# ShMonem/animSnapBases

Hardware: AMD Instinct MI355X
Metric: snapshots/sec (SVD+SPLOCS) for n_verts x n_frames; basis Frobenius err vs ref (higher is better)
Workload: dtype f64

## Files before the change

animsnapbases_amd/_lib.py:

```python
import ctypes
import os

import numpy as np

_HERE = os.path.dirname(os.path.abspath(__file__))
LIB_PATH = os.path.join(_HERE, "libasb_hip.so")

c_dp = ctypes.c_void_p
c_i64 = ctypes.c_int64
c_int = ctypes.c_int
c_dbl = ctypes.c_double

ASB_OK = 0
ERR_LIMIT = -4
DEFLATE_RESIDUAL, DEFLATE_PROJECT = 0, 1

PROTOTYPES = {
    "asb_abi_version": (c_int, []),
    "asb_create": (c_int, [c_int, ctypes.c_void_p, ctypes.POINTER(ctypes.c_void_p)]),
    "asb_destroy": (None, [ctypes.c_void_p]),
    "asb_last_error": (ctypes.c_char_p, [ctypes.c_void_p]),
    "asb_sync": (c_int, [ctypes.c_void_p]),
    "asb_prof_reset": (c_int, [ctypes.c_void_p, c_int]),
    "asb_prof_get": (c_int, [ctypes.c_void_p, ctypes.POINTER(c_i64), ctypes.POINTER(c_dbl)]),
# ... 98 lines not shown
    "asb_deflate_download_residual": (c_int, [ctypes.c_void_p, c_dp]),
    "asb_deflate_block_argmax": (c_int, [ctypes.c_void_p, c_int, c_dp, c_dp]),
    "asb_deflate_force_next": (c_int, [ctypes.c_void_p, c_i64]),
    "asb_components_post": (c_int, [ctypes.c_void_p, c_int, c_dbl, c_dp, c_dp]),
    "asb_orth_gram": (c_int, [ctypes.c_void_p, c_dp]),
    "asb_orth_apply": (c_int, [ctypes.c_void_p, c_dp, c_dp]),
    "asb_orth_refine": (c_int, [ctypes.c_void_p, c_dp]),
    "asb_orth_gram_get": (c_int, [ctypes.c_void_p, c_dp]),
    "asb_components_transform": (c_int, [ctypes.c_void_p, c_dp]),
    "asb_components_download": (c_int, [ctypes.c_void_p, c_dp]),
    "asb_components_upload": (c_int, [ctypes.c_void_p, c_dp, c_i64]),
    "asb_geodesic_setup": (c_int, [ctypes.c_void_p, c_int, c_int] + [c_dp] * 14),
    "asb_geodesic_solve": (c_int, [ctypes.c_void_p, c_dp, c_int, c_dbl, c_dp, c_dp]),
    "asb_geodesic_dense_setup": (c_int, [ctypes.c_void_p]),
    "asb_geodesic_bt_setup": (c_int, [ctypes.c_void_p, c_int, c_dp, c_dp, c_dp, c_dp, c_dp, c_dp, c_dp, c_dp]),
    "asb_deflate_apply_geodesic": (c_int, [ctypes.c_void_p, c_i64, c_dbl, c_dbl]),
    "asb_align_frames": (c_int, [ctypes.c_void_p, c_dp, c_i64, c_i64, c_int, c_dp]),
    "asb_pod_gram": (c_int, [ctypes.c_void_p, c_dp, c_dp]),
    "asb_pod_basis": (c_int, [ctypes.c_void_p, c_dp, c_dp, c_i64]),
    "asb_pod_project": (c_int, [ctypes.c_void_p, c_dp, c_dp]),
    "asb_components_truncate": (c_int, [ctypes.c_void_p, c_i64]),
    "asb_sym_tridiag": (c_int, [ctypes.c_void_p, c_dp, c_i64, c_dp, c_dp]),
    "asb_sym_backtransform": (c_int, [ctypes.c_void_p, c_dp, c_i64, c_dp, c_i64, c_dp]),
    "asb_snapshots_affine": (c_int, [ctypes.c_void_p, c_dbl, c_int, c_dp]),
    "asb_qr_apply": (c_int, [ctypes.c_void_p, c_dp]),
    "asb_deim_step": (c_int, [ctypes.c_void_p, c_i64, c_dp, ctypes.POINTER(c_i64), ctypes.POINTER(c_dbl)]),
    "asb_deim_row": (c_int, [ctypes.c_void_p, c_i64, c_dp]),
    "asb_recon_sweep": (c_int, [ctypes.c_void_p, c_int, c_dp, c_i64, c_dp, c_dp, c_dp]),
    "asb_heldout_upload": (c_int, [ctypes.c_void_p, c_dp, c_i64, c_i64, c_i64, c_i64, c_dp, c_int, c_dbl]),
    "asb_heldout_gram": (c_int, [ctypes.c_void_p, c_dp, c_dp]),
    "asb_heldout_factor": (c_int, [ctypes.c_void_p, c_dp, c_dp, ctypes.POINTER(c_i64)]),
    "asb_heldout_weights": (c_int, [ctypes.c_void_p, c_dp]),
    "asb_rows_gather": (c_int, [ctypes.c_void_p, c_int, c_dp, c_i64, c_dp, c_dp]),
    "asb_interp_sweep": (c_int, [ctypes.c_void_p, c_int, c_dp, c_dp, c_i64, c_dp, c_dp, c_i64, c_dp, c_dp, c_dp]),
    "asb_onmesh_mesh": (c_int, [ctypes.c_void_p, c_dp, c_i64, c_dp, c_dp, c_i64, c_i64]),
    "asb_onmesh_run": (c_int, [ctypes.c_void_p, c_int, c_i64, c_i64, c_i64, c_i64, c_int, c_dp, c_int, c_dbl, c_dbl,
                               c_dp, c_dp, c_dp, c_dp, c_dp, c_dp, c_dp]),
    "asb_cproj_setup": (c_int, [ctypes.c_void_p, c_int, c_i64, c_dp, c_dp, c_dp, c_dp]),
    "asb_cproj_run": (c_int, [ctypes.c_void_p, c_int, c_i64, c_i64, c_i64, c_dp, c_int, c_dbl, c_dbl, c_dbl, ctypes.c_void_p]),
    "asb_cforce_run": (c_int, [ctypes.c_void_p, c_int, c_i64, c_i64, c_i64, c_dp, c_int, c_dbl, c_dbl, c_dbl, c_i64, c_dp, c_dp, c_dp,
                               c_int, c_i64, ctypes.c_void_p]),
    "asb_splocs_begin": (c_int, [ctypes.c_void_p]),
    "asb_splocs_gram": (c_int, [ctypes.c_void_p, c_dp, c_dp, ctypes.POINTER(c_dbl)]),
    "asb_splocs_weights": (c_int, [ctypes.c_void_p, c_dp, c_dp, c_dp, c_dp]),
    "asb_splocs_admm": (c_int, [ctypes.c_void_p, c_dp, c_dbl, c_int]),
    "asb_splocs_admm_fields": (c_int, [ctypes.c_void_p, c_dp, c_dbl, c_dbl, c_dbl, c_dbl, c_int]),
    "asb_geodesic_cache_add": (c_int, [ctypes.c_void_p, c_dp, c_int, c_dbl, c_dp]),
    "asb_geodesic_cache_clear": (c_int, [ctypes.c_void_p]),
    "asb_splocs_objective": (c_int, [ctypes.c_void_p, c_dp, c_dp, ctypes.POINTER(c_dbl), ctypes.POINTER(c_dbl),
                                     ctypes.POINTER(c_dbl)]),
    "asb_splocs_results": (c_int, [ctypes.c_void_p, c_dp, c_dp]),
    "asb_test_eig3": (None, [c_dp, c_dp]),
    "asb_test_eig3_fast": (None, [c_dp, c_dp]),
    "asb_test_pick_cfg": (None, [c_i64, c_dp]),
    "asb_test_eig3_dev": (c_int, [ctypes.c_void_p, c_int, c_dp, c_i64, c_dp, c_i64]),
    "asb_test_deflate_step": (c_int, [ctypes.c_void_p, c_i64, c_dp, c_dbl, c_dp]),
    "asb_test_deflate_state": (c_int, [ctypes.c_void_p, c_dp, c_dp, c_dp, c_dp, c_dp, c_dp, c_dp, c_dp]),
    "asb_test_local_best": (c_int, [ctypes.c_void_p, c_i64, c_dp]),
    "asb_test_pick_records": (c_int, [ctypes.c_void_p, c_i64, c_dp, c_i64]),
    "asb_test_sketch_predict": (c_int, [ctypes.c_void_p, c_dp, c_dp, c_dp, c_i64, c_int, c_int, c_dp, ctypes.POINTER(c_i64),
                                        ctypes.POINTER(c_int)]),
    "asb_test_spd_inverse": (c_int, [ctypes.c_void_p, c_dp, c_i64, c_dp]),
    "asb_test_project_columns": (c_int, [ctypes.c_void_p, c_dp, c_i64, c_i64, c_int, c_dp, c_int, c_dp, c_i64]),
    "asb_test_gemm_nn": (c_int, [ctypes.c_void_p, c_dp, c_i64, c_dp, c_i64, c_dp, c_i64, c_i64, c_i64, c_i64, c_dbl, c_dbl, c_int,
                                 c_i64]),
    "asb_test_gemm_tn": (c_int, [ctypes.c_void_p, c_int, c_dp, c_i64, c_i64, c_dp, c_i64, c_i64, c_i64, c_i64, c_dp, c_i64, c_i64,
                                 c_i64, c_i64]),
    "asb_test_transpose": (c_int, [ctypes.c_void_p, c_dp, c_i64, c_i64, c_dp, c_i64]),
    "asb_test_sym_eig": (c_int, [ctypes.c_void_p, c_dp, c_i64, c_dp, c_dp, ctypes.POINTER(c_int)]),
    "asb_test_splocs_install": (c_int, [ctypes.c_void_p, c_dp, c_dp, c_dp]),
    "asb_test_splocs_state": (c_int, [ctypes.c_void_p, c_dp, c_dp, c_dp, c_dp, c_dp]),
    "asb_test_slab_gemm64": (c_int, [ctypes.c_void_p, c_dp, c_i64, c_dp, c_dp, c_i64, c_i64, c_dbl, c_dbl, c_int]),
    "asb_test_geodesic_field1": (c_int, [ctypes.c_void_p, c_i64, c_dp]),
    "asb_test_support_weights": (c_int, [ctypes.c_void_p, c_dp, c_i64, c_i64, c_i64, c_dbl, c_dbl, c_dp]),
    "asb_test_geodesic_cached": (c_int, [ctypes.c_void_p, c_i64, c_dp]),
}


class AsbLibraryError(RuntimeError):
    pass


_lib = None


def _preload_torch_hip_runtime():
    import importlib.util
    import sys
    if "torch" in sys.modules:
        return
    try:
        spec = importlib.util.find_spec("torch")
    except (ImportError, ValueError):
        spec = None
    if spec is None or not spec.origin:
        return
    libdir = os.path.join(os.path.dirname(spec.origin), "lib")
    for name in ("libamdhip64.so", "libamdhip64.so.7", "libamdhip64.so.6"):
        path = os.path.join(libdir, name)
        if os.path.exists(path):
            try:
                ctypes.CDLL(path, mode=ctypes.RTLD_GLOBAL)
            except OSError:
                pass
            return

# ... 35 lines not shown
```

animsnapbases_amd/csrc/asb_deflate.hip:

```cpp
#include "asb_kernels.h"

extern "C" void asb_test_eig3(const double* a6, double* out4) {
    eig3_top(a6[0], a6[1], a6[2], a6[3], a6[4], a6[5], out4[0], out4[1], out4[2], out4[3]);
}
extern "C" void asb_test_eig3_fast(const double* a6, double* out4) {
    eig3_top_fast(a6[0], a6[1], a6[2], a6[3], a6[4], a6[5], out4[0], out4[1], out4[2], out4[3]);
}
extern "C" void asb_test_pick_cfg(int64_t Fp, int* out5) {
    StreamCfg c{0, 0, 0, 0};
    out5[0] = pick_cfg(Fp, c) ? 1 : 0;
    out5[1] = c.T; out5[2] = c.E2; out5[3] = c.block; out5[4] = c.vpb;
}

static int stream_pass(asb_ctx* ctx, bool update, const double* wk, double* scal_k, const double* s,
                       double* ck) {
    StreamCfg c;
    if (!pick_cfg(ctx->Fp, c)) ASB_FAIL(ctx, ASB_ERR_LIMIT, "F = %lld too large (max 32768)", (long long)ctx->F);
    const int grid = stream_grid(ctx, c, ctx->n_loc);
    StreamArgs a{ctx->R, wk, scal_k, s, ck, ctx->energy, ctx->pmax, ctx->pidx, ctx->psum, (long long)ctx->n_loc, nullptr};
    size_t slot;
    int rc = prof_begin(ctx, slot);
    if (rc) return rc;
    launch_stream(ctx, c, update, grid, a);
    ASB_CHECK_LAUNCH(ctx);
    rc = prof_end(ctx, slot);
    if (rc) return rc;
    ctx->nblk = grid;
    return ASB_OK;
}

extern "C" int asb_deflate_begin(asb_ctx* ctx, int64_t K, int mode, int local_support) {
    if (!ctx) return ASB_ERR_ARG;
    if (!ctx->X) ASB_FAIL(ctx, ASB_ERR_ARG, "asb_deflate_begin: no snapshots uploaded");
    if (K < 1) ASB_FAIL(ctx, ASB_ERR_ARG, "asb_deflate_begin: K = %lld", (long long)K);
    if (mode != ASB_DEFLATE_RESIDUAL && mode != ASB_DEFLATE_PROJECT)
        ASB_FAIL(ctx, ASB_ERR_ARG, "asb_deflate_begin: unknown mode %d", mode);
    if (mode == ASB_DEFLATE_PROJECT && local_support)
        ASB_FAIL(ctx, ASB_ERR_ARG, "asb_deflate_begin: the projection mode is only valid for global support");
    ASB_HIP(ctx, hipSetDevice(ctx->dev));
    ctx->K = K;
    ctx->mode = mode;
    ctx->local = local_support;
    ctx->k_done = 0;
    ctx->n_panels = ctx->n_refresh = 0;
    ctx->n_spec_steps = ctx->n_spec_kept = 0;
    ctx->n_guess_panels = 0;
    ctx->n_coop_launches = ctx->max_read_kept = 0;
    ctx->n_sketch_runs = ctx->n_sketch_reads = 0;
    if (ctx->sk_counts) ASB_HIP(ctx, hipMemsetAsync(ctx->sk_counts, 0, 4 * sizeof(unsigned), ctx->stream));
    ctx->sketch_valid = false;
    ctx->sketch_run_off = false;
    ctx->read_by_score = ctx->last_by_score = false;
    ctx->rate_plain = ctx->rate_sketch = -1.0;
    ctx->mode_streak = 0;
    ctx->probe_after = 2;
    ctx->spec_budget = ASB_PANEL_COLS;
    ctx->fb_mark_reads = ctx->fb_mark_k = 0;
    ctx->k_switch = -1;
    {
// ... 376 lines not shown
```

animsnapbases_amd/csrc/asb_kernels.h:

```cpp
#pragma once
#include "asb_common.h"

#include <cmath>
#include <cstdlib>
#include <cstring>



template <int T, int E2, bool UPDATE>
__global__ __launch_bounds__((T >= 256 ? T : 256)) void k_stream(
    double* __restrict__ R, const double* __restrict__ wk, double* __restrict__ scal_k,
    const double* __restrict__ s, double* __restrict__ ck_out, double* __restrict__ energy,
    double* __restrict__ pmax, long long* __restrict__ pidx, double* __restrict__ psum,
    long long n_loc, int F2, const PanelState* __restrict__ panel) {
    if (panel != nullptr) {
        if (panel->done) return;
        if (panel->n_cand < n_loc) n_loc = panel->n_cand;
    }
    constexpr int BLOCK = (T >= 256 ? T : 256);
    constexpr int VPB = BLOCK / T;
    constexpr int NW = T / 64;
    const int tid = threadIdx.x;
    const int g = tid / T, t = tid % T;
    const int wig = t >> 6, lane = tid & 63;
// ... 158 lines not shown
__host__ __device__ inline void eig3_top_fast(double a00, double a01, double a02, double a11, double a12, double a22,
                                              double& lam, double& u0, double& u1, double& u2) {
    const double sc = fmax(fmax(fabs(a00), fabs(a11)), fmax(fabs(a22), fmax(fabs(a01), fmax(fabs(a02), fabs(a12)))));
    if (!(sc > 0.0) || !(sc < 1.0e300)) { eig3_top(a00, a01, a02, a11, a12, a22, lam, u0, u1, u2); return; }
    const double is = 1.0 / sc;
    const double b00 = a00 * is, b01 = a01 * is, b02 = a02 * is, b11 = a11 * is, b12 = a12 * is, b22 = a22 * is;
    const double q = (b00 + b11 + b22) / 3.0;
    const double p1 = b01 * b01 + b02 * b02 + b12 * b12;
    const double d0 = b00 - q, d1 = b11 - q, d2 = b22 - q;
    const double p = sqrt((d0 * d0 + d1 * d1 + d2 * d2 + 2.0 * p1) / 6.0);
    bool ok = p > 0.0;
    double l = q, x = 0.0, y = 0.0, z = 0.0;
    if (ok) {
        const double ip = 1.0 / p;
        const double c00 = d0 * ip, c11 = d1 * ip, c22 = d2 * ip, c01 = b01 * ip, c02 = b02 * ip, c12 = b12 * ip;
        double r = 0.5 * (c00 * (c11 * c22 - c12 * c12) - c01 * (c01 * c22 - c12 * c02) + c02 * (c01 * c12 - c11 * c02));
        r = fmin(1.0, fmax(-1.0, r));
        l = q + 2.0 * p * cos(acos(r) / 3.0);
        for (int it = 0; it < 3 && ok; ++it) {
            const double m00 = b00 - l, m11 = b11 - l, m22 = b22 - l;
            const double x0 = b01 * b12 - b02 * m11, y0 = b02 * b01 - m00 * b12, z0 = m00 * m11 - b01 * b01;
            const double x1 = b01 * m22 - b02 * b12, y1 = b02 * b02 - m00 * m22, z1 = m00 * b12 - b01 * b02;
            const double x2 = m11 * m22 - b12 * b12, y2 = b12 * b02 - b01 * m22, z2 = b01 * b12 - m11 * b02;
            const double n0 = x0 * x0 + y0 * y0 + z0 * z0, n1 = x1 * x1 + y1 * y1 + z1 * z1, n2 = x2 * x2 + y2 * y2 + z2 * z2;
            double nn;
            if (n0 >= n1 && n0 >= n2) { x = x0; y = y0; z = z0; nn = n0; }
            else if (n1 >= n2) { x = x1; y = y1; z = z1; nn = n1; }
            else { x = x2; y = y2; z = z2; nn = n2; }
            if (!(nn > 1.0e-20)) { ok = false; break; }
            const double inn = 1.0 / sqrt(nn);
            x *= inn; y *= inn; z *= inn;
            const double ln = x * (b00 * x + b01 * y + b02 * z) + y * (b01 * x + b11 * y + b12 * z) + z * (b02 * x + b12 * y + b22 * z);
            const bool settled = fabs(ln - l) <= 8.9e-16 * fabs(ln);
            l = ln;
            if (settled) break;
        }
    }
    if (ok) {
        const double r0 = b00 * x + b01 * y + b02 * z - l * x, r1 = b01 * x + b11 * y + b12 * z - l * y,
                     r2 = b02 * x + b12 * y + b22 * z - l * z;
        const double tr = b00 + b11 + b22 - l;
        const double mm = b00 * b11 - b01 * b01 + b00 * b22 - b02 * b02 + b11 * b22 - b12 * b12 - l * tr;
        const double disc = tr * tr - 4.0 * mm;
        const double l2 = 0.5 * (tr + sqrt(fmax(disc, 0.0)));
        ok = fmax(fabs(r0), fmax(fabs(r1), fabs(r2))) <= 1.0e-15 && l2 <= l * (1.0 - 1.0e-6);
    }
    if (!ok) { eig3_top(a00, a01, a02, a11, a12, a22, lam, u0, u1, u2); return; }
    const double m0 = fabs(x), m1 = fabs(y), m2 = fabs(z);
    const double lead = (m0 >= m1 && m0 >= m2) ? x : (m1 >= m2 ? y : z);
    if (lead < 0.0) { x = -x; y = -y; z = -z; }
    lam = l * sc; u0 = x; u1 = y; u2 = z;
}

__device__ inline void reduce_partials(const double* pmax, const long long* pidx, const double* psum,
                                int nblk, double* sh_d, long long* sh_i, double& be, long long& bi,
                                double& bs) {
    const int tid = threadIdx.x, nt = blockDim.x;
    double e = -1.0, s = 0.0;
    long long ix = 0x7fffffffffffffffLL;
    for (int b = tid; b < nblk; b += nt) {
        s += psum[b];
        if (am_better(pmax[b], pidx[b], e, ix)) {
            e = pmax[b];
            ix = pidx[b];
        }
    }
    sh_d[tid] = e;
    sh_d[nt + tid] = s;
    sh_i[tid] = ix;
    __syncthreads();
    for (int o = nt >> 1; o > 0; o >>= 1) {
        if (tid < o) {
            sh_d[nt + tid] += sh_d[nt + tid + o];
            if (am_better(sh_d[tid + o], sh_i[tid + o], sh_d[tid], sh_i[tid])) {
                sh_d[tid] = sh_d[tid + o];
                sh_i[tid] = sh_i[tid + o];
            }
        }
        __syncthreads();
    }
    be = sh_d[0];
    bi = sh_i[0];
    bs = sh_d[nt];
    __syncthreads();
}

static __global__ __launch_bounds__(256) void k_local_best(const double* __restrict__ R,
                                                    const double* pmax, const long long* pidx,
                                                    const double* psum, int nblk, long long v0,
                                                    int Fp, double* __restrict__ rec,
                                                    double* __restrict__ scal, long long k, long long forced,
                                                    long long n_loc) {
    __shared__ double sh_d[512];
    __shared__ long long sh_i[256];
    double be, bs;
    long long bi;
    reduce_partials(pmax, pidx, psum, nblk, sh_d, sh_i, be, bi, bs);
    if (forced >= 0) {
        const bool mine = forced >= v0 && forced < v0 + n_loc;
        be = mine ? 1.0e300 : -1.0;
        bi = mine ? forced - v0 : 0;
    }
    if (threadIdx.x == 0) {
        rec[0] = be;
        rec[1] = __longlong_as_double(v0 + bi);
        if (k > 0) scal[(k - 1) * 4 + 3] = bs;
// ... 217 lines not shown
```

animsnapbases_amd/csrc/asb_project.hip:

```cpp
#include "asb_kernels.h"

#include <algorithm>
#include <atomic>
#include <chrono>
#include <cstdlib>

typedef double d4 __attribute__((ext_vector_type(4)));

#define ASB_NBINS 2048

enum { SC_NORMX2 = 0, SC_E0MAX = 1, SC_EMAX = 2, SC_LO = 3, SC_HI = 4, SC_ABOVE = 5, SC_TAU = 6, SC_OVERFLOW = 7,
       SC_TAU_HI = 11, SC_TAU2 = 12, SC_BANDMAX = 13, SC_TAUG = 16, SC_GG = 24, SC_HH = 32,
       SC_TAU_DIV = 40, SC_DIV_SEED = 41 };
#define ASB_NG 6
__device__ __forceinline__ double guess_score(double ev, double m, double s, double g, double h) { return ev + g * m + h * s; }
__device__ __forceinline__ bool in_guess(double e, double ev, const double* __restrict__ sc) {
    const double m = e - ev, s = sqrt(fmax(m, 0.0) * fmax(ev, 0.0));
    bool in = false;
#pragma unroll
    for (int q = 0; q < ASB_NG; ++q) in = in || (guess_score(ev, m, s, sc[SC_GG + q], sc[SC_HH + q]) > sc[SC_TAUG + q]);
    return in;
}
static inline bool diverse_on(const asb_ctx* ctx) {
    return ctx->diverse && (!ctx->ev_valid || ctx->ev_cv2 > 0.5);
// ... 2085 lines not shown
    if (world > 16 || lds > 150 * 1024) return ASB_ERR_LIMIT;
    int rc;
    if ((rc = asb_alloc(ctx, &ctx->bam_idx, (size_t)256))) return rc;
    if (lds > 48 * 1024)
        ASB_HIP(ctx, hipFuncSetAttribute((const void*)k_global_tau, hipFuncAttributeMaxDynamicSharedMemorySize, (int)lds));
    hipLaunchKernelGGL(k_global_tau, dim3(1), dim3(1024), lds, ctx->stream, tab_dev, world, (long long)cap,
                       (long long)(ctx->m_target_eff ? ctx->m_target_eff : ctx->m_target) + 1, ctx->scalar_dev, ctx->bam_idx);
    ASB_CHECK_LAUNCH(ctx);
    long long h[16];
    if ((rc = fetch_words(ctx, ctx->bam_idx, world, h))) return rc;
    for (int r = 0; r < world; ++r) counts_out[r] = h[r];
    return ASB_OK;
}

__device__ __forceinline__ void coop_store(double* p, double v) { __hip_atomic_store(p, v, __ATOMIC_RELAXED, __HIP_MEMORY_SCOPE_AGENT); }
__device__ __forceinline__ double coop_load(const double* p) {
    return __hip_atomic_load(const_cast<double*>(p), __ATOMIC_RELAXED, __HIP_MEMORY_SCOPE_AGENT);
}

struct MultiArgs { long long kb[ASB_MAX_SUB]; int steps[ASB_MAX_SUB]; int spec_max[ASB_MAX_SUB]; int nsub; };
#define ASB_SENT_D 0xFFFFFFFFFFFFFFFFull
#define ASB_SENT_I (-1LL)

__device__ __forceinline__ unsigned long long coop_load_u64(const unsigned long long* p) {
    return __hip_atomic_load(const_cast<unsigned long long*>(p), __ATOMIC_RELAXED, __HIP_MEMORY_SCOPE_AGENT);
}
__device__ __forceinline__ void coop_store_u64(unsigned long long* p, unsigned long long v) {
    __hip_atomic_store(p, v, __ATOMIC_RELAXED, __HIP_MEMORY_SCOPE_AGENT);
}

__global__ __launch_bounds__(256) void k_panel_arm_multi(PanelState* __restrict__ panel, PanelState* __restrict__ sub,
                                                         const double* __restrict__ sc, double margin_rel, unsigned* __restrict__ coop_flags,
                                                         unsigned long long* __restrict__ words, int n_words, MultiArgs ma,
                                                         long long n_slots = -1) {
    for (int r = threadIdx.x; r < n_words; r += blockDim.x) words[r] = ASB_SENT_D;
    if (threadIdx.x < 4) coop_flags[threadIdx.x] = 0u;
    if (threadIdx.x != 0) return;
    if (n_slots >= 0) panel->n_cand = n_slots;
    panel->pad &= 1;
    panel->theta = panel->pad ? 1.0e300 : sc[SC_TAU];
    panel->margin = margin_rel * sc[SC_E0MAX];
    panel->done = 0;
    panel->committed = 0;
    panel->proven = -1;
    panel->spec_max = ma.spec_max[0];
    panel->spec_ok = ASB_PANEL_COLS;
    for (int sp = 0; sp < ASB_MAX_SUB; ++sp) {
        sub[sp] = *panel;
        sub[sp].spec_max = sp < ma.nsub ? ma.spec_max[sp] : 0;
    }
}

template <int NJ>
__global__ __launch_bounds__(256, (NJ > 16 ? 1 : 2)) void k_panel_multi(const double* __restrict__ R0, int F, int Fp,
                                                        double* __restrict__ W, double* __restrict__ scal, MultiArgs ma,
                                                        const PanelState* panel, PanelState* sub,
                                                        const long long* __restrict__ cand_idx, unsigned* __restrict__ bar,
                                                        unsigned long long* rec, unsigned long long* wbuf, unsigned long long* swbuf,
                                                        double* rows_out, int test_stall, int spec_rank) {
    constexpr int NQ = NJ / 4;
    __shared__ __attribute__((aligned(16))) double w_sh[NJ * 64 + 8];
    __shared__ double wv_e[4];
    __shared__ long long wv_i[4];
    __shared__ double sh_e[4];
    __shared__ int sh_i[4];
    __shared__ int sh_c[4];
    const int tid = threadIdx.x, lane = tid & 63, wv = tid >> 6;
    const int G = gridDim.x;
    const long long n_cand = panel->n_cand;
    if (n_cand > 4LL * G) {
        if (blockIdx.x == 0 && tid == 0) bar[2] = 1u;
        return;
    }
    const int Gact = n_cand > 0 ? (int)((n_cand + 3) / 4) : 1;
    if ((int)blockIdx.x >= Gact) return;
    const int WROW = Fp + 8;
    const double thr = panel->theta + panel->margin, e_floor = panel->margin;
    const bool overflow = panel->pad != 0;
    const long long s = (long long)blockIdx.x * 4 + wv;
    const bool have = s < n_cand && cand_idx[s] >= 0;
    double x[3][NJ];
    {
        const double* row = R0 + s * 3 * (long long)Fp;
#pragma unroll
        for (int d = 0; d < 3; ++d)
#pragma unroll
            for (int j = 0; j < NJ; ++j) {
                const int f = lane + 64 * j;
                x[d][j] = (have && f < Fp) ? row[(long long)d * Fp + f] : 0.0;
            }
    }
    if (spec_rank > 0) {
#pragma unroll
        for (int r3 = 0; r3 < 3; ++r3) {
            unsigned long long* sown = swbuf + ((size_t)r3 * G + blockIdx.x) * WROW;
            for (int f = tid; f < WROW; f += 256) coop_store_u64(sown + f, ASB_SENT_D);
        }
    }
    double g[6] = {0, 0, 0, 0, 0, 0};
#pragma unroll
    for (int j = 0; j < NJ; ++j) {
        const double a = x[0][j], b = x[1][j], c = x[2][j];
        g[0] += a * a; g[1] += a * b; g[2] += a * c; g[3] += b * b; g[4] += b * c; g[5] += c * c;
    }
    wave_sum_dpp<6>(g);
    unsigned long long* tlog = reinterpret_cast<unsigned long long*>(bar + 4);
    const long long spin_max = test_stall ? (1LL << 10) : (1LL << 20);
    int gstep = 0;
    bool aborted = false, ended = false;
    bool spec_now = false, spec_prev = false;
    int sp = 0;
    for (; sp < ma.nsub && !ended; ++sp) {
        const long long k0 = ma.kb[sp];
        const int steps = ma.steps[sp], spec_max = overflow ? 0 : ma.spec_max[sp];
        PanelState* st = sub + sp;
        int proven = -1, nrun = 0;
        for (int t = 0; t < steps; ++t, ++gstep) {
            const int ring = gstep % 3, ring_prev = (gstep + 2) % 3;
            if (blockIdx.x == 0 && tid == 0) tlog[gstep * 6 + 0] = wall_clock64();
            const double e = (g[0] + g[3]) + g[5];
            if (lane == 0) { wv_e[wv] = have ? e : -1.0; wv_i[wv] = have ? s : 0x7fffffffffffffffLL; }
            __builtin_amdgcn_s_waitcnt(0);
            __syncthreads();
            int ow = 0;
#pragma unroll
            for (int q = 1; q < 4; ++q)
                if (am_better(wv_e[q], wv_i[q], wv_e[ow], wv_i[ow])) ow = q;
            unsigned long long* myrec = rec + ((size_t)ring * G + blockIdx.x) * 2;
            if (tid == 0 && !(test_stall && (int)blockIdx.x == Gact - 1)) {
                const unsigned long long slot32 = wv_i[ow] > 0x7ffffffeLL ? 0x7fffffffull : (unsigned long long)wv_i[ow];
                coop_store(reinterpret_cast<double*>(myrec), wv_e[ow]);
                coop_store_u64(myrec + 1, slot32 | (spec_now && wv_e[ow] > 0.0 ? (1ull << 32) : 0ull));
            }
            if (blockIdx.x == 0 && tid == 0) tlog[gstep * 6 + 1] = wall_clock64();
            double lam = 0.0, u0 = 0.0, u1 = 0.0, u2 = 0.0;
            double be = -2.0;
            int bi = 0x7fffffff, dead = 0, better = 0;
            if (wv == ow) {
                if (wv_e[ow] > 0.0) {
                    eig3_top_fast(g[0], g[1], g[2], g[3], g[4], g[5], lam, u0, u1, u2);
                    double wn1[1] = {0.0};
#pragma unroll
                    for (int j = 0; j < NJ; ++j) {
                        const double wvv = u0 * x[0][j] + u1 * x[1][j] + u2 * x[2][j];
                        w_sh[lane + 64 * j] = wvv;
                        wn1[0] += wvv * wvv;
                    }
                    wave_sum_dpp<1>(wn1);
                    if (lane == 0) { w_sh[NJ * 64] = wn1[0]; w_sh[NJ * 64 + 1] = lam; }
                    if (spec_now) {
                        double* sw = reinterpret_cast<double*>(swbuf) + ((size_t)ring * G + blockIdx.x) * WROW;
#pragma unroll
                        for (int q = 0; q < NJ / 2; ++q) {
                            const int f2 = 2 * lane + 128 * q;
                            if (f2 < Fp) {
                                typedef double d2v __attribute__((ext_vector_type(2)));
                                const d2v v = *reinterpret_cast<const d2v*>(&w_sh[f2]);
                                asm volatile("global_store_dwordx4 %0, %1, off sc1" :: "v"(sw + f2), "v"(v) : "memory");
                            }
                        }
                        if (lane == 0) {
                            typedef double d2v __attribute__((ext_vector_type(2)));
                            const d2v hd2 = {wn1[0], lam};
                            asm volatile("global_store_dwordx4 %0, %1, off sc1" :: "v"(sw + Fp), "v"(hd2) : "memory");
                        }
                    }
                }
            } else {
                const unsigned long long* recs = rec + (size_t)ring * G * 2;
                const int p = (wv - (wv > ow ? 1 : 0)) * 64 + lane;
                for (int b = p; b < Gact; b += 192) {
                    unsigned long long eb, ib;
                    long long spins = 0;
                    for (;;) {
                        eb = coop_load_u64(recs + 2 * b);
                        ib = coop_load_u64(recs + 2 * b + 1);
                        if (eb != ASB_SENT_D && ib != (unsigned long long)ASB_SENT_I) break;
                        if ((++spins & 63) == 0 &&
                            (spins > spin_max || __hip_atomic_load(bar + 1, __ATOMIC_RELAXED, __HIP_MEMORY_SCOPE_AGENT))) { dead = 1; break; }
                    }
                    if (dead) break;
                    const double ebd = __longlong_as_double((long long)eb);
                    const int sl = (int)(ib & 0x7fffffffull);
                    const int ibs = sl == 0x7fffffff ? 0x7fffffff : 2 * sl + ((ib >> 32) & 1ull ? 0 : 1);
                    if (ebd > be || (ebd == be && ibs < bi)) { be = ebd; bi = ibs; }
                    if (ebd > wv_e[ow] || (ebd == wv_e[ow] && (long long)sl < wv_i[ow])) ++better;
                }
                const double em = wave_max_dpp(be);
                bi = wave_min_dpp(be == em ? bi : 0x7fffffff);
                be = em;
                better = wave_isum_dpp(better);
            }
            if (lane == 0) { sh_e[wv] = be; sh_i[wv] = bi; sh_c[wv] = better; }
            if (__syncthreads_or(dead)) { aborted = true; break; }
            be = sh_e[0]; bi = sh_i[0];
#pragma unroll
            for (int q = 1; q < 4; ++q)
                if (sh_e[q] > be || (sh_e[q] == be && sh_i[q] < bi)) { be = sh_e[q]; bi = sh_i[q]; }
            const bool win_spec = bi != 0x7fffffff && (bi & 1) == 0;
            if (bi != 0x7fffffff) bi >>= 1;
            const int bb = bi >> 2;
            const bool spec_mine = spec_now && wv_e[ow] > 0.0;
            spec_now = spec_rank > 0 && wv_e[ow] > 0.0 && (sh_c[0] + sh_c[1] + sh_c[2] + sh_c[3]) < spec_rank;
            if (blockIdx.x == 0 && tid == 0) tlog[gstep * 6 + 2] = wall_clock64();
            if (tid == 0) {
                unsigned long long* old = rec + ((size_t)ring_prev * G + blockIdx.x) * 2;
                coop_store_u64(old, ASB_SENT_D);
                coop_store_u64(old + 1, (unsigned long long)ASB_SENT_I);
            }
            if (spec_prev) {
                unsigned long long* sold = swbuf + ((size_t)ring_prev * G + blockIdx.x) * WROW;
#pragma unroll
                for (int q = 0; q < NQ; ++q) {
                    const int f = tid + 256 * q;
                    if (f < Fp) coop_store_u64(sold + f, ASB_SENT_D);
                }
                if (tid < 2) coop_store_u64(sold + Fp + tid, ASB_SENT_D);
            }
            spec_prev = spec_mine;
            {
                unsigned long long* wold = wbuf + (size_t)ring_prev * WROW;
                const int per = (WROW + Gact - 1) / Gact;
                const int f1 = ((int)blockIdx.x + 1) * per < WROW ? ((int)blockIdx.x + 1) * per : WROW;
                for (int f = (int)blockIdx.x * per + tid; f < f1; f += 256) coop_store_u64(wold + f, ASB_SENT_D);
            }
            if (!(be > thr) || bi >= n_cand) {
                if (proven < 0) proven = t;
                if (bi >= n_cand || !(be > e_floor) || t - proven >= spec_max) {
                    if (blockIdx.x == 0 && tid == 0) st->done = 1;
                    ended = true;
                    break;
                }
            }
            nrun = t + 1;
            unsigned long long* wb = win_spec ? swbuf + ((size_t)ring * G + bb) * WROW : wbuf + (size_t)ring * WROW;
            dead = 0;
            if (bb == (int)blockIdx.x && win_spec) {
            } else if (bb == (int)blockIdx.x) {
#pragma unroll
                for (int q = 0; q < NQ; ++q) {
                    const int f = tid + 256 * q;
                    if (f < Fp) coop_store(reinterpret_cast<double*>(wb) + f, w_sh[f]);
                }
                if (tid < 2) coop_store(reinterpret_cast<double*>(wb) + Fp + tid, w_sh[NJ * 64 + tid]);
            } else {
                unsigned long long tmp[NQ], hd = 0ull;
                long long spins = 0;
                for (;;) {
                    bool all = true;
#pragma unroll
                    for (int q = 0; q < NQ; ++q) {
                        const int f = tid + 256 * q;
                        tmp[q] = (f < Fp) ? coop_load_u64(wb + f) : 0ull;
                        all = all && tmp[q] != ASB_SENT_D;
                    }
                    if (tid < 2) { hd = coop_load_u64(wb + Fp + tid); all = all && hd != ASB_SENT_D; }
                    if (all) break;
                    if ((++spins & 63) == 0 &&
                        (spins > spin_max || __hip_atomic_load(bar + 1, __ATOMIC_RELAXED, __HIP_MEMORY_SCOPE_AGENT))) { dead = 1; break; }
                }
#pragma unroll
                for (int q = 0; q < NQ; ++q) w_sh[tid + 256 * q] = __longlong_as_double((long long)tmp[q]);
                if (tid < 2) w_sh[NJ * 64 + tid] = __longlong_as_double((long long)hd);
            }
            if (__syncthreads_or(dead)) { aborted = true; break; }
            if (blockIdx.x == 0 && tid == 0) tlog[gstep * 6 + 3] = wall_clock64();
            const double wn2 = w_sh[NJ * 64];
            if (bb == (int)blockIdx.x) {
                const long long k = k0 + t;
                for (int f = tid; f < Fp; f += 256) W[k * (long long)Fp + f] = w_sh[f];
                if (tid == 0) {
                    scal[k * 4 + 0] = sqrt(fmax(w_sh[NJ * 64 + 1], 0.0));
                    scal[k * 4 + 1] = wn2;
                    scal[k * 4 + 2] = __longlong_as_double(cand_idx[bi]);
                    st->e_win[t] = be;
                }
            }
            if (blockIdx.x == 0 && tid == 0) st->committed = t + 1;
            if (have) {
                double acc[3] = {0.0, 0.0, 0.0};
                constexpr int JB = NJ < 8 ? NJ : 8;
#pragma unroll
                for (int jb = 0; jb < NJ; jb += JB) {
                    double wj[JB];
#pragma unroll
                    for (int u = 0; u < JB; ++u) wj[u] = w_sh[lane + 64 * (jb + u)];
#pragma unroll
                    for (int u = 0; u < JB; ++u) {
                        acc[0] += x[0][jb + u] * wj[u]; acc[1] += x[1][jb + u] * wj[u]; acc[2] += x[2][jb + u] * wj[u];
                    }
                    __builtin_amdgcn_sched_barrier(0);
                }
                wave_sum_dpp<3>(acc);
#pragma unroll
                for (int d = 0; d < 3; ++d) acc[d] /= wn2;
#pragma unroll
                for (int q = 0; q < 6; ++q) g[q] = 0.0;
#pragma unroll
                for (int jb = 0; jb < NJ; jb += JB) {
                    double wj[JB];
#pragma unroll
                    for (int u = 0; u < JB; ++u) wj[u] = w_sh[lane + 64 * (jb + u)];
#pragma unroll
                    for (int u = 0; u < JB; ++u) {
                        const int j = jb + u;
                        const double a = x[0][j] - acc[0] * wj[u], b = x[1][j] - acc[1] * wj[u], c = x[2][j] - acc[2] * wj[u];
                        x[0][j] = a; x[1][j] = b; x[2][j] = c;
                        g[0] += a * a; g[1] += a * b; g[2] += a * c; g[3] += b * b; g[4] += b * c; g[5] += c * c;
                    }
                    __builtin_amdgcn_sched_barrier(0);
                }
                wave_sum_dpp<6>(g);
            }
            if (blockIdx.x == 0 && tid == 0) tlog[gstep * 6 + 4] = wall_clock64();
        }
        if (aborted) break;
        if (blockIdx.x == 0 && tid == 0) st->proven = proven < 0 ? nrun : proven;
        if (nrun < ASB_PANEL_COLS) ended = true;
    }
    if (aborted) {
        if (tid == 0) __hip_atomic_store(bar + 1, 1u, __ATOMIC_RELAXED, __HIP_MEMORY_SCOPE_AGENT);
        return;
    }
    if (blockIdx.x == 0 && tid == 0)
        for (int q = sp; q < ma.nsub; ++q) { sub[q].proven = 0; sub[q].done = 1; }
    if (rows_out != nullptr && have) {
        double* row = rows_out + s * 3 * (long long)Fp;
#pragma unroll
        for (int d = 0; d < 3; ++d)
#pragma unroll
            for (int j = 0; j < NJ; ++j) {
                const int f = lane + 64 * j;
                if (f < Fp) row[(long long)d * Fp + f] = x[d][j];
            }
    }
}

static int coop_buffers(asb_ctx* ctx, int* cgrid_all, size_t* n_words) {
    int rc;
    *cgrid_all = (int)((ctx->m_cap + 3) / 4);
    *n_words = (size_t)3 * *cgrid_all * 2 + (size_t)3 * (ctx->Fp + 8) + (size_t)3 * *cgrid_all * (ctx->Fp + 8);
    if ((rc = asb_alloc(ctx, &ctx->coop_bar, (size_t)4 + 2 * 64 * 6))) return rc;
    return asb_alloc(ctx, &ctx->coop_rec, *n_words);
}
constexpr int SPEC_W_RANK = 24;

template <int NJ>
static int launch_panel_multi(asb_ctx* ctx, int grid, const MultiArgs& ma, bool* launched, PanelState* sub, bool writeback) {
    int per_cu = 0;
    ASB_HIP(ctx, hipOccupancyMaxActiveBlocksPerMultiprocessor(&per_cu, (const void*)k_panel_multi<NJ>, 256, 0));
    if (per_cu < 1) { *launched = false; return ASB_OK; }
    if ((long long)per_cu * ctx->n_cu < grid) grid = per_cu * ctx->n_cu;
    unsigned long long* words = (unsigned long long*)ctx->coop_rec;
    hipLaunchKernelGGL(k_panel_multi<NJ>, dim3(grid), dim3(256), 0, ctx->stream, ctx->candR, (int)ctx->F, (int)ctx->Fp, ctx->W, ctx->scal,
                       ma, ctx->pstate, sub, ctx->cand_idx, ctx->coop_bar, words, words + (size_t)3 * grid * 2,
                       words + (size_t)3 * grid * 2 + (size_t)3 * (ctx->Fp + 8), writeback ? ctx->candR : (double*)nullptr,
                       ctx->coop_test_stall, SPEC_W_RANK);
    ASB_CHECK_LAUNCH(ctx);
    *launched = true;
    ctx->n_coop_launches++;
    return ASB_OK;
}

static int launch_panel_multi_any(asb_ctx* ctx, int grid, const MultiArgs& ma, bool* launched, PanelState* sub, bool writeback) {
    if (ctx->Fp <= 256) return launch_panel_multi<4>(ctx, grid, ma, launched, sub, writeback);
    if (ctx->Fp <= 512) return launch_panel_multi<8>(ctx, grid, ma, launched, sub, writeback);
    if (ctx->Fp <= 1024) return launch_panel_multi<16>(ctx, grid, ma, launched, sub, writeback);
    return launch_panel_multi<32>(ctx, grid, ma, launched, sub, writeback);
}
#define ASB_COOP_MAX_FP 2048
static bool coop_fits(const asb_ctx* ctx) { return ctx->panel_coop && ctx->Fp <= ASB_COOP_MAX_FP; }
static void print_multi_timeline(asb_ctx* ctx, int nsteps) {
    unsigned long long tl[64 * 6];
    (void)hipMemcpy(tl, ctx->coop_bar + 4, sizeof(tl), hipMemcpyDeviceToHost);
    for (int t = 0; t < 64 && t < nsteps; t += (nsteps > 16 ? 5 : 1))
        fprintf(stderr, "[asb]   step %2d: best+publish %.2f | poll+eigen %.2f | winner w %.2f | deflate+Gram %.2f | total %.2f us\n", t,
                (tl[t * 6 + 1] - tl[t * 6 + 0]) * 0.01, (tl[t * 6 + 2] - tl[t * 6 + 1]) * 0.01, (tl[t * 6 + 3] - tl[t * 6 + 2]) * 0.01,
                (tl[t * 6 + 4] - tl[t * 6 + 3]) * 0.01, (tl[t * 6 + 4] - tl[t * 6 + 0]) * 0.01);
}

struct PanelRunIn {
    long long k0 = 0;
    int steps = 0;
    int global_all = 0;
    int assembled = 0;
    int spec_max = 0;
    bool writeback = false;
    bool allow_coop = true;
};
struct PanelRunOut {
    int64_t committed = 0;
    long long proven = 0;
    bool coop_used = false;
};
static int panel_run(asb_ctx* ctx, const PanelRunIn& in, PanelRunOut* out) {
    if (!ctx || !ctx->candR || ctx->mode != ASB_DEFLATE_PROJECT || !out) return ASB_ERR_ARG;
    const long long k0 = in.k0;
    const int steps = in.steps;
    if (steps < 1 || steps > ASB_PANEL_COLS || k0 < 0 || k0 + steps > ctx->K)
        ASB_FAIL(ctx, ASB_ERR_ARG, "asb_panel_run: bad range k0=%lld steps=%d", (long long)k0, steps);
    const StreamCfg c = ctx->cfg;
    int rc;
    if ((rc = asb_alloc(ctx, &ctx->cand_c, (size_t)ASB_PANEL_COLS * ctx->m_cap * 3))) return rc;
    if ((rc = asb_alloc(ctx, &ctx->slab_scratch, (size_t)3 * ctx->Fp))) return rc;
    PanelState h;
    bool coop = false;
    for (bool allow_coop = in.allow_coop;; allow_coop = false) {
        int cgrid_all = 0;
        size_t n_words = 0;
        const bool want_coop = allow_coop && coop_fits(ctx);
        if (want_coop && (rc = coop_buffers(ctx, &cgrid_all, &n_words))) return rc;
        const long long spec_max = want_coop && !in.global_all ? in.spec_max : 0;
        hipLaunchKernelGGL(k_panel_arm, dim3(1), dim3(256), 0, ctx->stream, ctx->pstate, ctx->scalar_dev, in.global_all,
                           (long long)(in.assembled ? ctx->n_slots_host : -1), ASB_MARGIN_REL, want_coop ? ctx->coop_bar : (unsigned*)nullptr,
                           want_coop ? (unsigned long long*)ctx->coop_rec : (unsigned long long*)nullptr,
                           want_coop ? 3 * cgrid_all * 2 + 3 * ((int)ctx->Fp + 8) : 0,
                           0, spec_max);
        const int grid = stream_grid(ctx, c, ctx->m_cap);
        coop = false;
        if (want_coop) {
            MultiArgs ma{};
            ma.kb[0] = k0;
            ma.steps[0] = steps;
            ma.spec_max[0] = (int)spec_max;
            ma.nsub = 1;
            if ((rc = launch_panel_multi_any(ctx, cgrid_all, ma, &coop, ctx->pstate, in.writeback))) return rc;
        }
        if (in.assembled && !coop) {
            StreamArgs a{ctx->candR, nullptr, nullptr, nullptr, nullptr, ctx->cand_e, ctx->cpmax, ctx->cpidx, ctx->cpsum,
                         (long long)ctx->m_cap, ctx->pstate};
            launch_stream(ctx, c, false, grid, a);
// ... 1267 lines not shown
```

include/asb.h:

```cpp
#ifndef ASB_H
#define ASB_H

#include <stdint.h>

#ifdef __cplusplus
extern "C" {
#endif

#define ASB_ABI_VERSION 1

typedef struct asb_ctx asb_ctx;

typedef enum asb_status {
    ASB_OK = 0,
    ASB_ERR_ARG = -1,
    ASB_ERR_HIP = -2,
    ASB_ERR_NODEV = -3,
    ASB_ERR_LIMIT = -4,
    ASB_ERR_NUMERIC = -5
} asb_status;

int asb_abi_version(void);
#define ASB_STREAM_DEFAULT ((void*)(intptr_t)-1)
int asb_create(int device_id, void* hip_stream, asb_ctx** out);
// ... 145 lines not shown
int asb_pod_slices_basis(asb_ctx* ctx, int p, int64_t K, const double* VS_all_dev);
int asb_qr_apply_joint(asb_ctx* ctx, const double* G_dev);
int asb_snapshots_affine(asb_ctx* ctx, double inv_scale, int add_mean, const double* rowscale);
int asb_qr_apply(asb_ctx* ctx, const double* G_dev);
int asb_deim_step(asb_ctx* ctx, int64_t k, const double* coef, int64_t* idx_out, double* val_out);
int asb_deim_run(asb_ctx* ctx, int64_t* Pt_out, double* maxabs_out, int* solve_failed);
int asb_deim_block_residual(asb_ctx* ctx, int64_t k, int p, const double* coef, double* maxabs_out);
int asb_energy_block_argmax(asb_ctx* ctx, int p, int64_t* block_out, double* val_out);
int asb_deim_row(asb_ctx* ctx, int64_t gidx, double* row_out);

int asb_recon_sweep(asb_ctx* ctx, int which, const int64_t* ks, int64_t S, double* sums_out, double* max_out,
                    double* norms_out);
int asb_heldout_upload(asb_ctx* ctx, const double* Y, int64_t F, int64_t N_glob, int64_t v0, int64_t n_loc,
                       const double* massL, int subtract, double pre_scale_factor);
int asb_heldout_gram(asb_ctx* ctx, double* P_dev, double* G_dev);
int asb_heldout_factor(asb_ctx* ctx, const double* P_dev, const double* G_dev, int64_t* n_dropped);
int asb_heldout_weights(asb_ctx* ctx, double* W_out);

int asb_rows_gather(asb_ctx* ctx, int which, const int64_t* gidx, int64_t n, double* out, int* owned_out);
int asb_interp_sweep(asb_ctx* ctx, int which, const int64_t* rp, const int64_t* npt, int64_t S, const double* M, const double* B,
                     int64_t nb, double* sums_out, double* max_out, double* norms_out);

int asb_onmesh_mesh(asb_ctx* ctx, const int64_t* tris, int64_t n_tris, const int64_t* star_ptr, const int64_t* star_tri,
                    int64_t v0, int64_t n_loc);
int asb_onmesh_run(asb_ctx* ctx, int which, int64_t r, int64_t f0, int64_t f1, int64_t fj, int want_normals,
                   const double* inv_massL, int add_mean, double psf, double denom, double* accum_norm_out,
                   double* mesh_num_out, double* mesh_den_out, double* accum_angle_out, double* stats_out,
                   double* frame_err_out, double* angle_out);

int asb_cproj_setup(asb_ctx* ctx, int kind, int64_t n_elem, const int64_t* idx, const double* table, const int64_t* star_ptr,
                    const int64_t* star_idx);
int asb_cproj_run(asb_ctx* ctx, int which, int64_t f0, int64_t f1, int64_t fj, const double* inv_massL, int add_mean, double psf,
                  double sigma_min, double sigma_max, double* out_dev);
int asb_cforce_run(asb_ctx* ctx, int which, int64_t f0, int64_t f1, int64_t fj, const double* inv_massL, int add_mean, double psf,
                   double sigma_min, double sigma_max, int64_t n_rows, const int64_t* indptr, const int64_t* indices,
                   const double* data, int accumulate, int64_t chunk_frames, double* out_dev);

int asb_splocs_begin(asb_ctx* ctx);
int asb_splocs_gram(asb_ctx* ctx, double* P_dev, double* M_dev, double* normX2_local);
int asb_splocs_weights(asb_ctx* ctx, const double* P_dev, const double* M_dev,
                       int64_t* centre_idx, double* centre_val);
int asb_splocs_admm(asb_ctx* ctx, const double* Lambda, double rho, int n_iter);
int asb_splocs_admm_fields(asb_ctx* ctx, const int64_t* slots, double lambda, double dmin, double dmax, double rho, int n_iter);
int asb_splocs_objective(asb_ctx* ctx, const double* P_dev, const double* M_dev, double* wp,
                         double* gm, double* sparsity_local);
int asb_splocs_results(asb_ctx* ctx, double* C_out, double* W_out);

int asb_test_tridiag_eig(asb_ctx* ctx, const double* d, const double* e, int64_t n, int64_t k, double* lam_desc, double* Z,
                         int64_t* n_bad);
int asb_test_jacobi_rows(asb_ctx* ctx, const double* A, int64_t nv, int64_t m, double* U, double* sig, int64_t* sweeps);
int asb_test_chol_tinv(asb_ctx* ctx, const double* G, int64_t K, double* Tt);
void asb_test_eig3(const double* a6, double* out4);
void asb_test_eig3_fast(const double* a6, double* out4);
void asb_test_pick_cfg(int64_t Fp, int* out5);
int asb_test_eig3_dev(asb_ctx* ctx, int fast, const double* a6, int64_t n, double* out4, int64_t out_len);
int asb_test_deflate_step(asb_ctx* ctx, int64_t k, const double* w, double wn2, const double* s);
int asb_test_deflate_state(asb_ctx* ctx, double* energy, double* pmax, int64_t* pidx, double* psum, int64_t* counts, double* scal,
                           double* W, double* R);
int asb_test_local_best(asb_ctx* ctx, int64_t k, double* rec);
int asb_test_pick_records(asb_ctx* ctx, int64_t k, const double* recs, int64_t n_rec);
int asb_test_sketch_predict(asb_ctx* ctx, const double* cols, const double* wn2, const double* E, int64_t n, int r, int steps,
                            double* scores, int64_t* pred, int* status);
int asb_test_spd_inverse(asb_ctx* ctx, const double* A_host, int64_t n, double* Ainv_host);
int asb_test_project_columns(asb_ctx* ctx, const double* W_host, int64_t ldw, int64_t k0, int ncols, const double* col_scale_host,
                             int path, double* out_host, int64_t out_cols);
int asb_test_gemm_nn(asb_ctx* ctx, const double* A, int64_t lda, const double* B, int64_t ldb, double* C, int64_t ldc, int64_t M,
                     int64_t N, int64_t Kc, double alpha, double beta, int tri, int64_t c_len);
int asb_test_gemm_tn(asb_ctx* ctx, int form, const double* X, int64_t ldx, int64_t sx, const double* Y, int64_t ldy, int64_t R,
                     int64_t I, int64_t J, double* out, int64_t so_i, int64_t so_j, int64_t out_len, int64_t I_split);
int asb_test_transpose(asb_ctx* ctx, const double* in, int64_t rows, int64_t cols, double* out, int64_t out_len);
int asb_test_sym_eig(asb_ctx* ctx, const double* A, int64_t n, double* lam, double* V, int* status);
int asb_test_splocs_install(asb_ctx* ctx, const double* C, const double* W, const double* U);
int asb_test_splocs_state(asb_ctx* ctx, double* U, double* Lambda, double* G, double* Ginv, double* c);
int asb_test_slab_gemm64(asb_ctx* ctx, const double* A, int64_t lda, const double* Z, double* out, int64_t M, int64_t Kc,
                         double alpha, double beta, int nct);
int asb_test_geodesic_field1(asb_ctx* ctx, int64_t src, double* phi_out);
int asb_test_support_weights(asb_ctx* ctx, const double* phi, int64_t n, int64_t v0, int64_t n_loc, double dmin, double dmax,
                             double* s_out);
int asb_test_geodesic_cached(asb_ctx* ctx, int64_t slot, double* out);

#ifdef __cplusplus
}
#endif
#endif
```

Baseline: 468,600.

## Defer panel row deflation using Gram downdate to shorten step critical path

In the cooperative panel kernel, each step now computes only the row dots and a cheap rank-one downdate of the 3x3 Gram to publish the candidate energy. The full row update and exact Gram recomputation are deferred into the next step, after the publish barrier, so they overlap with cross-block polling. The exact pass still runs right away when the downdated energy falls below a sixteenth of its previous value (cancellation risk) or on the last step. w_sh is double-buffered so the deferred pass can read the previous direction. The cost is extra shared memory and a published energy that comes from the downdate rather than an exact recompute.

```diff
diff --git a/animsnapbases_amd/_lib.py b/animsnapbases_amd/_lib.py
--- a/animsnapbases_amd/_lib.py
+++ b/animsnapbases_amd/_lib.py
@@ -174,6 +174,7 @@
     "asb_splocs_results": (c_int, [ctypes.c_void_p, c_dp, c_dp]),
     "asb_test_eig3": (None, [c_dp, c_dp]),
     "asb_test_eig3_fast": (None, [c_dp, c_dp]),
+    "asb_test_gram_downdate": (None, [c_dp, c_dbl, c_dp, c_dp]),
     "asb_test_pick_cfg": (None, [c_i64, c_dp]),
     "asb_test_eig3_dev": (c_int, [ctypes.c_void_p, c_int, c_dp, c_i64, c_dp, c_i64]),
     "asb_test_deflate_step": (c_int, [ctypes.c_void_p, c_i64, c_dp, c_dbl, c_dp]),
diff --git a/animsnapbases_amd/csrc/asb_deflate.hip b/animsnapbases_amd/csrc/asb_deflate.hip
--- a/animsnapbases_amd/csrc/asb_deflate.hip
+++ b/animsnapbases_amd/csrc/asb_deflate.hip
@@ -5,6 +5,14 @@
 }
 extern "C" void asb_test_eig3_fast(const double* a6, double* out4) {
     eig3_top_fast(a6[0], a6[1], a6[2], a6[3], a6[4], a6[5], out4[0], out4[1], out4[2], out4[3]);
+}
+extern "C" void asb_test_gram_downdate(const double* g6, double wn2, const double* c3, double* out8) {
+    const double g[6] = {g6[0], g6[1], g6[2], g6[3], g6[4], g6[5]}, c[3] = {c3[0], c3[1], c3[2]};
+    double gd[6], e_new;
+    const bool exact_due = gram_downdate(g, wn2, c, gd, e_new);
+    for (int q = 0; q < 6; ++q) out8[q] = gd[q];
+    out8[6] = e_new;
+    out8[7] = exact_due ? 1.0 : 0.0;
 }
 extern "C" void asb_test_pick_cfg(int64_t Fp, int* out5) {
     StreamCfg c{0, 0, 0, 0};
diff --git a/animsnapbases_amd/csrc/asb_kernels.h b/animsnapbases_amd/csrc/asb_kernels.h
--- a/animsnapbases_amd/csrc/asb_kernels.h
+++ b/animsnapbases_amd/csrc/asb_kernels.h
@@ -234,6 +234,14 @@
     lam = l * sc; u0 = x; u1 = y; u2 = z;
 }
 
+__host__ __device__ inline bool gram_downdate(const double (&g)[6], double wn2, const double (&c)[3], double (&gd)[6], double& e_new) {
+    gd[0] = g[0] - wn2 * c[0] * c[0]; gd[1] = g[1] - wn2 * c[0] * c[1]; gd[2] = g[2] - wn2 * c[0] * c[2];
+    gd[3] = g[3] - wn2 * c[1] * c[1]; gd[4] = g[4] - wn2 * c[1] * c[2]; gd[5] = g[5] - wn2 * c[2] * c[2];
+    const double e = (g[0] + g[3]) + g[5], ed = (gd[0] + gd[3]) + gd[5];
+    e_new = fmax(ed, 0.0);
+    return !(ed >= e * 0.0625);
+}
+
 __device__ inline void reduce_partials(const double* pmax, const long long* pidx, const double* psum,
                                 int nblk, double* sh_d, long long* sh_i, double& be, long long& bi,
                                 double& bs) {
diff --git a/animsnapbases_amd/csrc/asb_project.hip b/animsnapbases_amd/csrc/asb_project.hip
--- a/animsnapbases_amd/csrc/asb_project.hip
+++ b/animsnapbases_amd/csrc/asb_project.hip
@@ -2161,6 +2161,45 @@
 }
 
 template <int NJ>
+__device__ __forceinline__ void panel_row_dots(const double (&x)[3][NJ], const double* w_sh, int lane, double (&acc)[3]) {
+    constexpr int JB = NJ < 8 ? NJ : 8;
+    acc[0] = acc[1] = acc[2] = 0.0;
+#pragma unroll
+    for (int jb = 0; jb < NJ; jb += JB) {
+        double wj[JB];
+#pragma unroll
+        for (int u = 0; u < JB; ++u) wj[u] = w_sh[lane + 64 * (jb + u)];
+#pragma unroll
+        for (int u = 0; u < JB; ++u) {
+            acc[0] += x[0][jb + u] * wj[u]; acc[1] += x[1][jb + u] * wj[u]; acc[2] += x[2][jb + u] * wj[u];
+        }
+        __builtin_amdgcn_sched_barrier(0);
+    }
+    wave_sum_dpp<3>(acc);
+}
+template <int NJ>
+__device__ __forceinline__ void panel_row_update(double (&x)[3][NJ], const double* w_sh, int lane, const double (&acc)[3], double (&g)[6]) {
+    constexpr int JB = NJ < 8 ? NJ : 8;
+#pragma unroll
+    for (int q = 0; q < 6; ++q) g[q] = 0.0;
+#pragma unroll
+    for (int jb = 0; jb < NJ; jb += JB) {
+        double wj[JB];
+#pragma unroll
+        for (int u = 0; u < JB; ++u) wj[u] = w_sh[lane + 64 * (jb + u)];
+#pragma unroll
+        for (int u = 0; u < JB; ++u) {
+            const int j = jb + u;
+            const double a = x[0][j] - acc[0] * wj[u], b = x[1][j] - acc[1] * wj[u], c = x[2][j] - acc[2] * wj[u];
+            x[0][j] = a; x[1][j] = b; x[2][j] = c;
+            g[0] += a * a; g[1] += a * b; g[2] += a * c; g[3] += b * b; g[4] += b * c; g[5] += c * c;
+        }
+        __builtin_amdgcn_sched_barrier(0);
+    }
+    wave_sum_dpp<6>(g);
+}
+
+template <int NJ>
 __global__ __launch_bounds__(256, (NJ > 16 ? 1 : 2)) void k_panel_multi(const double* __restrict__ R0, int F, int Fp,
                                                         double* __restrict__ W, double* __restrict__ scal, MultiArgs ma,
                                                         const PanelState* panel, PanelState* sub,
@@ -2168,7 +2207,7 @@
                                                         unsigned long long* rec, unsigned long long* wbuf, unsigned long long* swbuf,
                                                         double* rows_out, int test_stall, int spec_rank) {
     constexpr int NQ = NJ / 4;
-    __shared__ __attribute__((aligned(16))) double w_sh[NJ * 64 + 8];
+    __shared__ __attribute__((aligned(16))) double w_sh2[2][NJ * 64 + 8];
     __shared__ double wv_e[4];
     __shared__ long long wv_i[4];
     __shared__ double sh_e[4];
@@ -2218,6 +2257,9 @@
     int gstep = 0;
     bool aborted = false, ended = false;
     bool spec_now = false, spec_prev = false;
+    bool pending = false;
+    double acc[3] = {0.0, 0.0, 0.0};
+    double e_pub = (g[0] + g[3]) + g[5];
     int sp = 0;
     for (; sp < ma.nsub && !ended; ++sp) {
         const long long k0 = ma.kb[sp];
@@ -2226,9 +2268,10 @@
         int proven = -1, nrun = 0;
         for (int t = 0; t < steps; ++t, ++gstep) {
             const int ring = gstep % 3, ring_prev = (gstep + 2) % 3;
+            const double* w_old = w_sh2[(gstep + 1) & 1];
+            double* w_sh = w_sh2[gstep & 1];
             if (blockIdx.x == 0 && tid == 0) tlog[gstep * 6 + 0] = wall_clock64();
-            const double e = (g[0] + g[3]) + g[5];
-            if (lane == 0) { wv_e[wv] = have ? e : -1.0; wv_i[wv] = have ? s : 0x7fffffffffffffffLL; }
+            if (lane == 0) { wv_e[wv] = have ? e_pub : -1.0; wv_i[wv] = have ? s : 0x7fffffffffffffffLL; }
             __builtin_amdgcn_s_waitcnt(0);
             __syncthreads();
             int ow = 0;
@@ -2242,6 +2285,11 @@
                 coop_store_u64(myrec + 1, slot32 | (spec_now && wv_e[ow] > 0.0 ? (1ull << 32) : 0ull));
             }
             if (blockIdx.x == 0 && tid == 0) tlog[gstep * 6 + 1] = wall_clock64();
+            if (pending) {
+                panel_row_update<NJ>(x, w_old, lane, acc, g);
+                pending = false;
+            }
+            if (blockIdx.x == 0 && tid == 0) tlog[gstep * 6 + 2] = wall_clock64();
             double lam = 0.0, u0 = 0.0, u1 = 0.0, u2 = 0.0;
             double be = -2.0;
             int bi = 0x7fffffff, dead = 0, better = 0;
@@ -2311,7 +2359,7 @@
             const int bb = bi >> 2;
             const bool spec_mine = spec_now && wv_e[ow] > 0.0;
             spec_now = spec_rank > 0 && wv_e[ow] > 0.0 && (sh_c[0] + sh_c[1] + sh_c[2] + sh_c[3]) < spec_rank;
-            if (blockIdx.x == 0 && tid == 0) tlog[gstep * 6 + 2] = wall_clock64();
+            if (blockIdx.x == 0 && tid == 0) tlog[gstep * 6 + 3] = wall_clock64();
             if (tid == 0) {
                 unsigned long long* old = rec + ((size_t)ring_prev * G + blockIdx.x) * 2;
                 coop_store_u64(old, ASB_SENT_D);
@@ -2373,7 +2421,7 @@
                 if (tid < 2) w_sh[NJ * 64 + tid] = __longlong_as_double((long long)hd);
             }
             if (__syncthreads_or(dead)) { aborted = true; break; }
-            if (blockIdx.x == 0 && tid == 0) tlog[gstep * 6 + 3] = wall_clock64();
+            if (blockIdx.x == 0 && tid == 0) tlog[gstep * 6 + 4] = wall_clock64();
             const double wn2 = w_sh[NJ * 64];
             if (bb == (int)blockIdx.x) {
                 const long long k = k0 + t;
@@ -2386,42 +2434,21 @@
                 }
             }
             if (blockIdx.x == 0 && tid == 0) st->committed = t + 1;
-            if (have) {
-                double acc[3] = {0.0, 0.0, 0.0};
-                constexpr int JB = NJ < 8 ? NJ : 8;
-#pragma unroll
-                for (int jb = 0; jb < NJ; jb += JB) {
-                    double wj[JB];
-#pragma unroll
-                    for (int u = 0; u < JB; ++u) wj[u] = w_sh[lane + 64 * (jb + u)];
-#pragma unroll
-                    for (int u = 0; u < JB; ++u) {
-                        acc[0] += x[0][jb + u] * wj[u]; acc[1] += x[1][jb + u] * wj[u]; acc[2] += x[2][jb + u] * wj[u];
-                    }
-                    __builtin_amdgcn_sched_barrier(0);
+            const bool last = t + 1 == steps && (sp + 1 == ma.nsub || steps < ASB_PANEL_COLS);
+            if (have && !(last && rows_out == nullptr)) {
+                panel_row_dots<NJ>(x, w_sh, lane, acc);
+#pragma unroll
+                for (int d = 0; d < 3; ++d) acc[d] /= wn2;
+                double gd[6];
+                const bool exact_due = gram_downdate(g, wn2, acc, gd, e_pub);
+                if (exact_due || last) {
+                    panel_row_update<NJ>(x, w_sh, lane, acc, g);
+                    e_pub = (g[0] + g[3]) + g[5];
+                } else {
+                    pending = true;
                 }
-                wave_sum_dpp<3>(acc);
-#pragma unroll
-                for (int d = 0; d < 3; ++d) acc[d] /= wn2;
-#pragma unroll
-                for (int q = 0; q < 6; ++q) g[q] = 0.0;
-#pragma unroll
-                for (int jb = 0; jb < NJ; jb += JB) {
-                    double wj[JB];
-#pragma unroll
-                    for (int u = 0; u < JB; ++u) wj[u] = w_sh[lane + 64 * (jb + u)];
-#pragma unroll
-                    for (int u = 0; u < JB; ++u) {
-                        const int j = jb + u;
-                        const double a = x[0][j] - acc[0] * wj[u], b = x[1][j] - acc[1] * wj[u], c = x[2][j] - acc[2] * wj[u];
-                        x[0][j] = a; x[1][j] = b; x[2][j] = c;
-                        g[0] += a * a; g[1] += a * b; g[2] += a * c; g[3] += b * b; g[4] += b * c; g[5] += c * c;
-                    }
-                    __builtin_amdgcn_sched_barrier(0);
-                }
-                wave_sum_dpp<6>(g);
-            }
-            if (blockIdx.x == 0 && tid == 0) tlog[gstep * 6 + 4] = wall_clock64();
+            }
+            if (blockIdx.x == 0 && tid == 0) tlog[gstep * 6 + 5] = wall_clock64();
         }
         if (aborted) break;
         if (blockIdx.x == 0 && tid == 0) st->proven = proven < 0 ? nrun : proven;
@@ -2483,9 +2510,10 @@
     unsigned long long tl[64 * 6];
     (void)hipMemcpy(tl, ctx->coop_bar + 4, sizeof(tl), hipMemcpyDeviceToHost);
     for (int t = 0; t < 64 && t < nsteps; t += (nsteps > 16 ? 5 : 1))
-        fprintf(stderr, "[asb]   step %2d: best+publish %.2f | poll+eigen %.2f | winner w %.2f | deflate+Gram %.2f | total %.2f us\n", t,
+        fprintf(stderr, "[asb]   step %2d: best+publish %.2f | shadow pass %.2f | poll+eigen %.2f | winner w %.2f | dots+downdate %.2f | "
+                        "total %.2f us\n", t,
                 (tl[t * 6 + 1] - tl[t * 6 + 0]) * 0.01, (tl[t * 6 + 2] - tl[t * 6 + 1]) * 0.01, (tl[t * 6 + 3] - tl[t * 6 + 2]) * 0.01,
-                (tl[t * 6 + 4] - tl[t * 6 + 3]) * 0.01, (tl[t * 6 + 4] - tl[t * 6 + 0]) * 0.01);
+                (tl[t * 6 + 4] - tl[t * 6 + 3]) * 0.01, (tl[t * 6 + 5] - tl[t * 6 + 4]) * 0.01, (tl[t * 6 + 5] - tl[t * 6 + 0]) * 0.01);
 }
 
 struct PanelRunIn {
diff --git a/include/asb.h b/include/asb.h
--- a/include/asb.h
+++ b/include/asb.h
@@ -221,6 +221,7 @@
 int asb_test_chol_tinv(asb_ctx* ctx, const double* G, int64_t K, double* Tt);
 void asb_test_eig3(const double* a6, double* out4);
 void asb_test_eig3_fast(const double* a6, double* out4);
+void asb_test_gram_downdate(const double* g6, double wn2, const double* c3, double* out8);
 void asb_test_pick_cfg(int64_t Fp, int* out5);
 int asb_test_eig3_dev(asb_ctx* ctx, int fast, const double* a6, int64_t n, double* out4, int64_t out_len);
 int asb_test_deflate_step(asb_ctx* ctx, int64_t k, const double* w, double wn2, const double* s);
```

Measured after the change: 461,500 (median of 2 runs). No clear change (-1.5%).
